# georghess/neurad-studio

Measured on NVIDIA H100. Metric: rays/sec (camera+lidar), higher is better.
Workload: dtype f32

## Files before the change

### neurad-studio_b200/csrc/b200nerf.cu

```cuda
#include <cuda_runtime.h>

#include <cstdio>
#include <cstring>
#include <new>
#include <string>
#include <vector>

#include "../../include/b200nerf.h"
#include "nff_device.h"
#include "nff_lane.h"
#include "rgb_decoder.cuh"
#include "modules.cuh"
#include "lidar_eval.cuh"
#include "lidar_loss.cuh"
#include "image_metrics.cuh"
#include "camera_rays.h"

using namespace nff;

static thread_local std::string g_err;
static int fail(int code, const std::string& msg) {
  g_err = msg;
  return code;
}
// ... 171 lines not shown
  constexpr int kPatchesPerUnit = kLaneThreads / 32;
  return lane_unit_ray(P, patch / kPatchesPerUnit, (int)(patch % kPatchesPerUnit) * 32 + lane_, ray_out);
}

#ifndef NFF_SAMPLE_CTAS
#define NFF_SAMPLE_CTAS 2
#endif
template <int LAYOUT, bool ACTORS, bool TRACED, bool EDIT>
__global__ void __launch_bounds__(kLaneThreads, NFF_SAMPLE_CTAS) nff_sample_lane_kernel(const __grid_constant__ RenderParams P,
                                                                                        float* __restrict__ scratch,
                                                                                        float* __restrict__ handoff) {
  const int tid = threadIdx.x, warp = __shfl_sync(0xffffffffu, (int)(threadIdx.x >> 5), 0), lane_ = tid & 31;
  const LaneScratch sc = lane_scratch_of(scratch, blockIdx.x);
  __shared__ float e0_tab[kS0 + 1];
  const bool shared_edges = !P.rays.nears && !P.rays.fars;
  if (shared_edges) {
    if (tid <= kS0) e0_tab[tid] = lane_round0_edge(P.samp, tid);
    __syncthreads();
  }
  constexpr int kPPU = kLaneThreads / 32;
  const int64_t n_patches = lane_patches(P);
  const int64_t full_rounds = n_patches / kPPU / gridDim.x;
  const int64_t r0 = full_rounds * gridDim.x * kPPU, rest = n_patches - r0;
  const int64_t p0 = r0 + rest * blockIdx.x / gridDim.x, p1 = r0 + rest * (blockIdx.x + 1) / gridDim.x;
  for (int64_t it = 0;; ++it) {
    int64_t patch;
    if (it < full_rounds) {
      patch = (it * gridDim.x + blockIdx.x) * kPPU + warp;
    } else {
      patch = p0 + warp + (it - full_rounds) * kPPU;
      if (patch >= p1) break;
    }
    int64_t ray;
    const bool active = lane_patch_ray(P, patch, lane_, &ray);
    const LaneRay R = lane_ray_setup<ACTORS, EDIT>(P, sc, tid, ray);
    float* col = active ? handoff + ray : sc.bins2 + tid;
    sample_ray_lane<LAYOUT, ACTORS, TRACED>(P, sc, R, tid, ray, active, col, active ? P.n_rays : (int64_t)kLaneThreads,
                                            shared_edges ? e0_tab : nullptr);
  }
}
template <int LAYOUT>
static auto sample_lane_kernel(bool actors, bool traced, bool edit) {
  if (edit) return traced ? nff_sample_lane_kernel<LAYOUT, true, true, true> : nff_sample_lane_kernel<LAYOUT, true, false, true>;
  return traced ? nff_sample_lane_kernel<LAYOUT, true, true, false>
         : actors ? nff_sample_lane_kernel<LAYOUT, true, false, false>
                  : nff_sample_lane_kernel<LAYOUT, false, false, false>;
}

template <int LAYOUT, bool EDIT>
__global__ void __launch_bounds__(kLaneThreads, kLaneCtasPerSm) nff_shade_lane_kernel(const __grid_constant__ RenderParams P,
                                                                                      float* __restrict__ scratch,
                                                                                      const float* __restrict__ handoff) {
  extern __shared__ __align__(128) unsigned char smem_shade[];
  TcShared* tcs = reinterpret_cast<TcShared*>(smem_shade);
  const int tid = threadIdx.x, warp = __shfl_sync(0xffffffffu, (int)(threadIdx.x >> 5), 0), group = warp >> 2;
  tc_stage_weights(*tcs, P.main_mlp_nn, tid, kLaneThreads, true);
  tc::fence_async_smem();
  __syncthreads();
  MlpLaneTc mlp;
  mlp.t = tcs;
  mlp.panel_ = reinterpret_cast<float*>(smem_shade + kTcBytes);
  mlp.bar_id = 1 + group;
  const LaneScratch sc = lane_scratch_of(scratch, blockIdx.x);
  mlp.sh_tcnn = LAYOUT;
  constexpr int kPPU = kLaneThreads / 32;
  const int64_t n_patches = lane_patches(P);
  const int64_t full_rounds = n_patches / kPPU / gridDim.x;
  const int64_t r0 = full_rounds * gridDim.x * kPPU;
  const int64_t rest_groups = (n_patches - r0 + 3) / 4;
  const int64_t g0 = rest_groups * blockIdx.x / gridDim.x, g1 = rest_groups * (blockIdx.x + 1) / gridDim.x;
  for (int64_t it = 0;; ++it) {
    int64_t patch;
    if (it < full_rounds) {
      patch = (it * gridDim.x + blockIdx.x) * kPPU + warp;
    } else {
      const int64_t gu = g0 + group + (it - full_rounds) * (kLaneThreads / 128);
      if (gu >= g1) break;
      patch = r0 + gu * 4 + (warp & 3);
    }
    int64_t ray;
    const bool active = lane_patch_ray(P, patch, tid & 31, &ray);
    const LaneRay R = lane_ray_setup<true, EDIT>(P, sc, tid, ray);
    shade_ray_lane<MlpLaneTc, LAYOUT>(P, sc, R, mlp, tid, ray, active, handoff + ray, P.n_rays);
  }
}

template <bool EDIT>
__global__ void __launch_bounds__(kLaneThreads, kLaneCtasPerSm) nff_render_lane_kernel(const __grid_constant__ RenderParams P,
                                                                          float* __restrict__ scratch) {
  extern __shared__ __align__(128) unsigned char smem_lane[];
  TcShared* tcs = reinterpret_cast<TcShared*>(smem_lane);
  const int tid = threadIdx.x, warp = __shfl_sync(0xffffffffu, (int)(threadIdx.x >> 5), 0), group = warp >> 2;
  tc_stage_weights(*tcs, P.main_mlp_nn, tid, kLaneThreads, true);
  tc::fence_async_smem();
  __syncthreads();
  MlpLaneTc mlp;
  mlp.t = tcs;
  mlp.panel_ = reinterpret_cast<float*>(smem_lane + kTcBytes);
  mlp.bar_id = 1 + group;
  const LaneScratch sc = lane_scratch_of(scratch, blockIdx.x);
  for (int64_t unit = blockIdx.x; unit < lane_units(P); unit += gridDim.x) {
    int64_t ray;
    const bool active = lane_unit_ray(P, unit, tid, &ray);
    render_ray_lane<MlpLaneTc, 0, EDIT>(P, sc, mlp, tid, ray, active);
  }
}

__global__ void lidar_decode_kernel(const float* __restrict__ mlp, const float* __restrict__ feats, int fdim,
                                    int64_t n, float* __restrict__ intensity, float* __restrict__ drop) {
  __shared__ __align__(16) float w[kLidarMlpFloats];
  for (int i = threadIdx.x; i < kLidarMlpFloats; i += blockDim.x) w[i] = mlp[i];
  __syncthreads();
  int64_t r = (int64_t)blockIdx.x * blockDim.x + threadIdx.x;
  if (r >= n) return;
  float x[kNff + kApp];
#pragma unroll
  for (int i = 0; i < kNff + kApp; ++i) x[i] = i < fdim ? feats[r * fdim + i] : 0.f;
  float h[kHidden], h2[kHidden], o[2];
  dense<kNff + kApp, kHidden, kHidden, true>(w + kOffLidW0, w + kOffLidB0, x, h);
  dense<kHidden, kHidden, kHidden, true>(w + kOffLidW1, w + kOffLidB1, h, h2);
  dense<kHidden, 2, kLidOutP, false>(w + kOffLidW2, w + kOffLidB2, h2, o);
  if (intensity) intensity[r] = 1.0f / (1.0f + expf(-o[0]));
  if (drop) drop[r] = o[1];
}

__global__ void hashgrid_fwd_kernel(Grid g, const float* __restrict__ x, float* __restrict__ out,
                                    int32_t* __restrict__ indices, int64_t n_points) {
  int64_t i = (int64_t)blockIdx.x * blockDim.x + threadIdx.x;
  if (i >= n_points * g.L) return;
  int64_t p = i / g.L;
  int l = (int)(i % g.L);
  Cell c = grid_cell(x[3 * p], x[3 * p + 1], x[3 * p + 2], g.res[l]);
  uint32_t r[8];
  cell_rows(c, g.mask, r);
  if (indices) {
#pragma unroll
    for (int k = 0; k < 8; ++k) indices[(p * g.L + l) * 8 + k] = (int32_t)(r[k] + (uint32_t)l * g.T);
  }
  const float* base = g.table + (size_t)l * g.T * g.F;
  for (int f = 0; f < g.F; ++f) {
    float v[8];
#pragma unroll
    for (int k = 0; k < 8; ++k) v[k] = __ldg(base + (size_t)r[k] * g.F + f);
    out[p * g.L * g.F + l * g.F + f] = trilerp(v, c);
  }
}

template <int D>
__global__ void tcnn_hashgrid_fwd_kernel(Grid g, const float* __restrict__ x, float* __restrict__ out, int64_t n) {
  const int64_t i = (int64_t)blockIdx.x * blockDim.x + threadIdx.x;
  if (i >= n) return;
// ... 1750 lines not shown
  const Step steps[10] = {
      {features, nullptr, lo[0], H, W},
      {lo[0], nullptr, lo[1], H, W}, {lo[1], lo[0], lo[2], H, W},
      {lo[2], nullptr, lo[1], H, W}, {lo[1], lo[2], lo[0], H, W},
      {lo[0], nullptr, hi[0], H, W},
      {hi[0], nullptr, hi[1], HO, WO}, {hi[1], hi[0], hi[2], HO, WO},
      {hi[2], nullptr, hi[1], HO, WO}, {hi[1], hi[2], rgb, HO, WO},
  };
  for (int layer = 0; layer < 10; ++layer) {
    const Step& s = steps[layer];
    if (int e = b200nerf_rgb_decode_layer(c, layer, s.in, s.res, s.out, batch, s.h, s.w, impl, stream)) return e;
  }
  return 0;
}

int b200nerf_set_peer_outputs(b200nerf_ctx* c, const b200nerf_peer_outputs* peers) {
  REQUIRE(c, "ctx is NULL");
  if (!peers || peers->n_peers == 0) {
    c->peers = b200nerf_peer_outputs{};
    return 0;
  }
  REQUIRE(peers->n_peers > 0 && peers->n_peers <= B200NERF_MAX_PEERS, "n_peers must be in [1, 16]");
  REQUIRE(peers->self_rank >= -1 && peers->self_rank < peers->n_peers, "self_rank out of range");
  REQUIRE(peers->row_offset >= 0, "negative row_offset");
  for (int p = 0; p < peers->n_peers; ++p) {
    if (p == peers->self_rank) continue;
    REQUIRE(peers->features[p] && peers->depth[p] && peers->accumulation[p], "NULL peer buffer");
  }
  c->peers = *peers;
  return 0;
}

int b200nerf_set_param_stream(b200nerf_ctx* c, void* stream) {
  REQUIRE(c, "ctx is NULL");
  c->param_stream = (cudaStream_t)stream;
  return 0;
}

int b200nerf_set_mlp_mode(b200nerf_ctx* c, int mode) {
  REQUIRE(c, "ctx is NULL");
  REQUIRE(mode >= 0 && mode <= 3, "render mode: 0 = warp-per-ray + CUDA-core fp32, 1 = warp-per-ray + wgmma, 2 = ray-per-lane + wgmma, 3 = ray-per-lane in two kernels (sampling, shading)");
  c->mlp_mode = mode;
  return 0;
}

int b200nerf_check_status(b200nerf_ctx* c) {
  REQUIRE(c, "ctx is NULL");
  if (!c->d_status) return 0;
  DeviceGuard g(c->device);
  int st = 0;
  CUDA_TRY(cudaMemcpy(&st, c->d_status, sizeof(int), cudaMemcpyDeviceToHost));
  if (st != 0) {
    cudaMemset(c->d_status, 0, sizeof(int));
    return fail(B200NERF_ERR_CUDA, "device-side failure flag set (tensor-core pipeline timed out, code " + std::to_string(st) + ")");
  }
  return 0;
}

int b200nerf_hashgrid_fwd(b200nerf_ctx* c, const b200nerf_grid_desc* desc, const float* table, const float* x,
                          float* out, int32_t* indices, int64_t n_points, void* stream) {
  REQUIRE(c && desc, "NULL argument");
  REQUIRE(desc->features_per_level >= 1 && desc->features_per_level <= 8, "features_per_level must be in [1,8]");
  if (n_points == 0) return 0;
  REQUIRE(table && x && out, "NULL argument");
  DeviceGuard g(c->device);
  Grid gr{};
  if (int e = make_grid(desc, table, &gr)) return e;
  if (indices && (uint64_t)gr.L * gr.T > (1ull << 31))
    return fail(B200NERF_ERR_UNSUPPORTED, "row indices of more than 2^31 table rows do not fit int32");
  int64_t n = n_points * gr.L;
  hashgrid_fwd_kernel<<<(unsigned)((n + 255) / 256), 256, 0, (cudaStream_t)stream>>>(gr, x, out, indices, n_points);
  CUDA_TRY(cudaGetLastError());
  return 0;
}

int b200nerf_tcnn_hashgrid_fwd(b200nerf_ctx* c, const b200nerf_tcnn_grid_desc* desc, const float* params, const float* x,
                               float* out, int64_t n_points, void* stream) {
  REQUIRE(c && desc, "NULL argument");
  REQUIRE(desc->features_per_level >= 1 && desc->features_per_level <= 8, "features_per_level must be in [1,8]");
  REQUIRE(desc->n_input_dims == 3 || desc->n_input_dims == 4, "n_input_dims must be 3 or 4");
  if (n_points == 0) return 0;
  REQUIRE(params && x && out, "NULL argument");
  DeviceGuard g(c->device);
  Grid gr{};
  if (int e = make_tcnn_grid(desc, params, desc->n_input_dims, &gr)) return e;
  const unsigned blocks = (unsigned)((n_points + 127) / 128);
  if (desc->n_input_dims == 3)
    tcnn_hashgrid_fwd_kernel<3><<<blocks, 128, 0, (cudaStream_t)stream>>>(gr, x, out, n_points);
  else
    tcnn_hashgrid_fwd_kernel<4><<<blocks, 128, 0, (cudaStream_t)stream>>>(gr, x, out, n_points);
  CUDA_TRY(cudaGetLastError());
  return 0;
}

int b200nerf_sh4_fwd(b200nerf_ctx* c, const float* dirs, float* out, int64_t n, void* stream) {
  REQUIRE(c, "NULL argument");
  if (n == 0) return 0;
  REQUIRE(dirs && out, "NULL argument");
  DeviceGuard g(c->device);
  sh4_fwd_kernel<<<(unsigned)((n + 255) / 256), 256, 0, (cudaStream_t)stream>>>(dirs, out, n);
  CUDA_TRY(cudaGetLastError());
  return 0;
}

int b200nerf_pdf_resample(b200nerf_ctx* c, const float* weights, const float* bins, const float* u, int n_rays,
                          int s_old, int s_new, float hist_pad, float* new_bins, float* cdf, int32_t* inds,
// ... 316 lines not shown
```

### neurad-studio_b200/csrc/nff_device.h

```cpp
#pragma once
#include "nff_params.h"
#include "simt.h"

#ifndef NFF_G_PROP
#define NFF_G_PROP 1
#endif
#ifndef NFF_G_ACT
#define NFF_G_ACT 2
#endif
#ifndef NFF_ILP
#define NFF_ILP 2
#endif
#ifndef NFF_F4_UNROLL
#define NFF_F4_UNROLL 2
#endif
#ifndef NFF_FAST_RCP
#define NFF_FAST_RCP 1
#endif
#ifndef NFF_PARITY_STD
#define NFF_PARITY_STD 0
#endif
#ifndef NFF_PARITY_LERP
#define NFF_PARITY_LERP 0
#endif
// ... 726 lines not shown
struct MlpFfma {
  const float* w;
  template <class WS>
  NFF_D void run(WS& ws, const float dir[3], float& sdf, float* feat) const {
    const int ln = lane();
    const float* mlp = w;
    float mac[kGeoOutP];
    dense_panel<kGeoIn, kHidden, kHidden>(mlp + kOffGeoW0, mlp + kOffGeoB0, ws.act, mac);
#pragma unroll
    for (int i = 0; i < kHidden; ++i) ws.act[i][ln] = fmaxf(mac[i], 0.0f);
    dense_panel<kHidden, kNff + 1, kGeoOutP>(mlp + kOffGeoW1, mlp + kOffGeoB1, ws.act, mac);
    sdf = mac[0];
    float geo[kNff];
#pragma unroll
    for (int i = 0; i < kNff; ++i) {
      geo[i] = mac[i + 1];
      ws.act[i][ln] = geo[i];
    }
    {
      float shv[kSh];
      sh4(dir[0], dir[1], dir[2], shv);
#pragma unroll
      for (int i = 0; i < kSh; ++i) ws.act[kNff + i][ln] = shv[i];
    }
    dense_panel<kNff + kSh, kHidden, kHidden>(mlp + kOffFeatW0, mlp + kOffFeatB0, ws.act, mac);
#pragma unroll
    for (int i = 0; i < kHidden; ++i) ws.act[i][ln] = fmaxf(mac[i], 0.0f);
    dense_panel<kHidden, kHidden, kHidden>(mlp + kOffFeatW1, mlp + kOffFeatB1, ws.act, mac);
#pragma unroll
    for (int i = 0; i < kHidden; ++i) ws.act[i][ln] = fmaxf(mac[i], 0.0f);
    dense_panel<kHidden, kNff, kNff>(mlp + kOffFeatW2, mlp + kOffFeatB2, ws.act, mac);
#pragma unroll
    for (int i = 0; i < kNff; ++i) feat[i] = geo[i] + mac[i];
  }
};

#if defined(__CUDACC__)
}
#include "tc_mlp.cuh"
namespace nff {
constexpr int kTcLayers = 5;
constexpr int kTcPitch = tc::stage_pitch(48);
constexpr int kTcStageFloats = 128 * kTcPitch;
struct TcShared {
  float b[2 * 32 * (32 + 32 + 48 + 32 + 32)];
  float bias[kTcLayers][32];
  float w_sdf[32];
  float b_sdf;
};
constexpr int kTcBytes = (sizeof(TcShared) + 127) / 128 * 128;
constexpr size_t tc_smem_bytes(int threads) { return (size_t)kTcBytes + (size_t)(threads / 128) * kTcStageFloats * sizeof(float); }
NFF_D constexpr int tc_layer_k(int l) { return l == 2 ? 48 : 32; }
NFF_D constexpr int tc_layer_off(int l) { return l == 0 ? 0 : l == 1 ? 2048 : l == 2 ? 4096 : l == 3 ? 7168 : 9216; }

NFF_D void tc_stage_weights(TcShared& t, const float* NFF_RESTRICT nn, int tid, int nthreads, bool chained = false) {
  const int w_off[kTcLayers] = {kNnGeoW0, kNnGeoW1 + kHidden , kNnFeatW0, kNnFeatW1, kNnFeatW2};
  const int b_off[kTcLayers] = {kNnGeoB0, kNnGeoB1 + 1, kNnFeatB0, kNnFeatB1, kNnFeatB2};
#pragma unroll
  for (int l = 0; l < kTcLayers; ++l) {
    const int K = tc_layer_k(l);
    float* hi = t.b + tc_layer_off(l);
    tc::stage_b_tile(hi, hi + 32 * K, nn + w_off[l], 32, K, 32, K, tid, nthreads, chained && l > 0 ? 32 : 0);
    for (int i = tid; i < 32; i += nthreads) t.bias[l][i] = nn[b_off[l] + i];
  }
  for (int i = tid; i < 32; i += nthreads) t.w_sdf[i] = nn[kNnGeoW1 + i];
  if (tid == 0) t.b_sdf = nn[kNnGeoB1];
}

struct MlpTc {
  const TcShared* t;
  float* stage;
  int bar_id;

  template <int K>
  NFF_D void layer(int l, const float* x, float* out) {
    const float* hi = t->b + tc_layer_off(l);
    const int id = bar_id;
    tc::tile_layer<48, 32>(stage, kTcPitch, x, K, hi, hi + 32 * K, out, [id] { asm volatile("bar.sync %0, 128;" ::"r"(id) : "memory"); });
#pragma unroll
    for (int i = 0; i < 32; ++i) out[i] += t->bias[l][i];
  }

  template <class WS>
  NFF_D void run(WS& ws, const float dir[3], float& sdf, float* feat) {
    const int ln = lane();
    float x[kNff + kSh], h[kHidden];
#pragma unroll
    for (int i = 0; i < kGeoIn; ++i) x[i] = ws.act[i][ln];
    layer<32>(0, x, h);
    float s = t->b_sdf;
#pragma unroll
    for (int i = 0; i < kHidden; ++i) {
      h[i] = fmaxf(h[i], 0.0f);
      s = fmaf(h[i], t->w_sdf[i], s);
    }
    sdf = s;
    layer<32>(1, h, x);
    sh4(dir[0], dir[1], dir[2], x + kNff);
    layer<48>(2, x, h);
#pragma unroll
    for (int i = 0; i < kHidden; ++i) h[i] = fmaxf(h[i], 0.0f);
    float h2[kHidden];
    layer<32>(3, h, h2);
#pragma unroll
    for (int i = 0; i < kHidden; ++i) h2[i] = fmaxf(h2[i], 0.0f);
    layer<32>(4, h2, h);
#pragma unroll
    for (int i = 0; i < kNff; ++i) feat[i] = x[i] + h[i];
  }
};
#endif

template <class WS, class Mlp>
NFF_D void render_ray(const RenderParams& P, WS& ws, Mlp& mlp, int64_t ray, bool active) {
  const Sampling& sp = P.samp;
  const int ln = lane();
// ... 127 lines not shown
```

### neurad-studio_b200/csrc/nff_lane.h

```cpp
#pragma once
#include "nff_device.h"

namespace nff {

#ifndef NFF_LANE_THREADS
#define NFF_LANE_THREADS 512
#endif
#ifndef NFF_F4_WEIGHTS
#define NFF_F4_WEIGHTS 0
#endif
constexpr int kLaneThreads = NFF_LANE_THREADS;
constexpr int kLaneCtasPerSm = 512 / kLaneThreads;
constexpr int kCandFloats = 16;
constexpr int kLaneMaxCand = 32;

struct LaneScratch {
  float* w;
  float* bins1;
  float* bins2;
  float* cand;
};
NFF_HD size_t lane_scratch_floats_per_cta() {
  return (size_t)kLaneThreads * (kS0 + (kS1 + 1) + (kS2 + 1) + kLaneMaxCand * kCandFloats);
}
// ... 227 lines not shown
  int k = 1;
  double run = (double)fdiv(fadd(sc.w[tid], pad_each), tot);
  float c_km1 = 0.0f, c_k = fminf(1.0f, (float)run);
  float w_next = sc.w[(size_t)kLaneThreads + tid];
#pragma unroll 1
  for (int i = 0; i <= S_new; ++i) {
    const float u = ldg(io.u_tab + i);
    while (k <= S && c_k <= u) {
      ++k;
      c_km1 = c_k;
      if (k <= S) {
        const float wk = w_next;
        w_next = sc.w[(size_t)(k < S ? k : S - 1) * kLaneThreads + tid];
        run += (double)fdiv(fadd(wk, pad_each), tot);
        c_k = fminf(1.0f, (float)run);
      }
    }
    const int above = k > S ? S : k;
    const float b0 = edge(k - 1), b1 = edge(above);
    float t = nan_to_num(fdiv(fsub(u, c_km1), fsub(k > S ? c_km1 : c_k, c_km1)));
    t = fminf(fmaxf(t, 0.0f), 1.0f);
    const float nb = fadd(b0, fmul(t, fsub(b1, b0)));
    io.bins_out[(size_t)i * io.bins_stride] = nb;
    if (TRACED && io.tr_inds) io.tr_inds[ray * (S_new + 1) + i] = k;
    if (TRACED && io.tr_bins_s) io.tr_bins_s[ray * (S_new + 1) + i] = nb;
    if (TRACED && io.tr_bins_e) io.tr_bins_e[ray * (S_new + 1) + i] = to_euclid(nb, s_near, s_far, sp);
  }
  return depth_acc;
}

struct MlpLaneFfma {
  static constexpr int kPitch = kLaneThreads;
  const float* w;
  float* panel_;
  int sh_tcnn = 0;
  NFF_D float* panel() const { return panel_; }
  NFF_D void run(const float* x, const float dir[3], float& sdf, float* feat, int ) const {
    float h[kHidden], go[kNff + 1], in2[kNff + kSh], h2[kHidden];
    dense<kGeoIn, kHidden, kHidden, true>(w + kOffGeoW0, w + kOffGeoB0, x, h);
    dense<kHidden, kNff + 1, kGeoOutP, false>(w + kOffGeoW1, w + kOffGeoB1, h, go);
    sdf = go[0];
#pragma unroll
    for (int i = 0; i < kNff; ++i) in2[i] = go[i + 1];
    if (sh_tcnn) sh4_tcnn(dir[0], dir[1], dir[2], in2 + kNff); else sh4(dir[0], dir[1], dir[2], in2 + kNff);
    dense<kNff + kSh, kHidden, kHidden, true>(w + kOffFeatW0, w + kOffFeatB0, in2, h);
    dense<kHidden, kHidden, kHidden, true>(w + kOffFeatW1, w + kOffFeatB1, h, h2);
    dense<kHidden, kNff, kNff, false>(w + kOffFeatW2, w + kOffFeatB2, h2, h);
#pragma unroll
    for (int i = 0; i < kNff; ++i) feat[i] = in2[i] + h[i];
  }
};

#if defined(__CUDACC__)
constexpr int kLanePanelPitch = kLaneThreads + 8;
constexpr int kLanePanelRows = kGeoIn + kSh + 1;
constexpr size_t lane_tc_smem_bytes() { return (size_t)kTcBytes + sizeof(float) * kLanePanelRows * kLanePanelPitch; }
struct MlpLaneTc {
  static constexpr int kPitch = kLanePanelPitch;
  const TcShared* t;
  float* panel_;
  int bar_id;
  int sh_tcnn = 0;
  NFF_D float* panel() const { return panel_; }
  NFF_D void group_sync() const { asm volatile("bar.sync %0, 128;" ::"r"(bar_id) : "memory"); }

  NFF_D static uint32_t b_desc_lo() {
    extern __shared__ __align__(128) unsigned char nff_lane_smem[];
    return tc::smem_desc_lo(tc::smem_u32(nff_lane_smem + offsetof(TcShared, b)), 128u);
  }

  template <int KS, int K, int OFF>
  NFF_D static void half_mma(float* acc, const float* a) {
    uint32_t ah[4 * KS], al[4 * KS];
#pragma unroll
    for (int i = 0; i < 4 * KS; ++i) {
      const float h = tc::tf32_hi(a[i]);
      ah[i] = __float_as_uint(h);
      al[i] = __float_as_uint(a[i] - h);
    }
    constexpr uint32_t sbo = (uint32_t)(K / 4) * 128u;
    constexpr uint32_t hi_off = (uint32_t)OFF * 4u / 16u, lo_off = (uint32_t)(OFF + 32 * K) * 4u / 16u;
    const uint32_t b_desc = b_desc_lo();
    tc::wg_fence();
#pragma unroll
    for (int ks = 0; ks < KS; ++ks) {
      const uint32_t adv = (uint32_t)(ks * 2 * 128) / 16u;
      const uint64_t dh = tc::smem_desc_of(b_desc + hi_off + adv, sbo), dl = tc::smem_desc_of(b_desc + lo_off + adv, sbo);
      tc::wgmma_tf32<32>(acc, ah + 4 * ks, dh);
      tc::wgmma_tf32<32>(acc, al + 4 * ks, dh);
      tc::wgmma_tf32<32>(acc, ah + 4 * ks, dl);
    }
    tc::wg_commit();
    tc::wg_wait<0>();
    tc::reg_fence(acc, 16);
#pragma unroll
    for (int i = 0; i < 4 * KS; ++i) asm volatile("" : "+r"(ah[i]), "+r"(al[i])::"memory");
  }
  NFF_D static void chain(float* a, const float* acc) {
#pragma unroll
    for (int j = 0; j < 4; ++j) {
      a[4 * j + 0] = acc[4 * j + 0];
      a[4 * j + 1] = acc[4 * j + 2];
      a[4 * j + 2] = acc[4 * j + 1];
      a[4 * j + 3] = acc[4 * j + 3];
    }
  }
  NFF_D static void load_a(float* a, const float* p, int q, int ks0, int n) {
#pragma unroll
    for (int i = 0; i < n; ++i) {
      const float* r = p + (8 * (ks0 + i) + q) * kPitch;
      a[4 * i + 0] = r[0];
      a[4 * i + 1] = r[8];
      a[4 * i + 2] = r[4 * kPitch];
      a[4 * i + 3] = r[4 * kPitch + 8];
    }
  }
  NFF_D static void bias_init(float* acc, const float* bias, int q) {
#pragma unroll
    for (int j = 0; j < 4; ++j) {
      const float2 b = *reinterpret_cast<const float2*>(bias + 8 * j + 2 * q);
      acc[4 * j + 0] = acc[4 * j + 2] = b.x;
      acc[4 * j + 1] = acc[4 * j + 3] = b.y;
    }
  }
  NFF_D static void relu(float* acc) {
#pragma unroll
    for (int i = 0; i < 16; ++i) acc[i] = fmaxf(acc[i], 0.0f);
  }

  NFF_D void run(const float* , const float dir[3], float& sdf, float* feat, int tid) {
    float* col = panel_ + tid;
    {
      float shv[kSh];
      if (sh_tcnn) sh4_tcnn(dir[0], dir[1], dir[2], shv); else sh4(dir[0], dir[1], dir[2], shv);
#pragma unroll
      for (int i = 0; i < kSh; ++i) col[(kGeoIn + i) * kPitch] = shv[i];
    }
    group_sync();
    const int ln = tid & 31, q = ln & 3;
    float* const fr = panel_ + (tid & ~127) + 16 * ((tid >> 5) & 3) + (ln >> 2);
#pragma unroll 1
    for (int h = 0; h < 2; ++h) {
      float* const p = fr + 64 * h;
      float a[16], acc[16];
      load_a(a, p, q, 0, 4);
      bias_init(acc, t->bias[0], q);
      half_mma<4, 32, tc_layer_off(0)>(acc, a);
      relu(acc);
      float s0 = 0.0f, s1 = 0.0f;
#pragma unroll
      for (int j = 0; j < 4; ++j) {
        const float2 w = *reinterpret_cast<const float2*>(t->w_sdf + 8 * j + 2 * q);
        s0 = fmaf(acc[4 * j + 0], w.x, fmaf(acc[4 * j + 1], w.y, s0));
        s1 = fmaf(acc[4 * j + 2], w.x, fmaf(acc[4 * j + 3], w.y, s1));
      }
      s0 += __shfl_xor_sync(0xffffffffu, s0, 1);
      s1 += __shfl_xor_sync(0xffffffffu, s1, 1);
      s0 += __shfl_xor_sync(0xffffffffu, s0, 2);
      s1 += __shfl_xor_sync(0xffffffffu, s1, 2);
      if (q == 0) {
        p[(kGeoIn + kSh) * kPitch] = s0 + t->b_sdf;
        p[(kGeoIn + kSh) * kPitch + 8] = s1 + t->b_sdf;
      }
      chain(a, acc);
      bias_init(acc, t->bias[1], q);
      half_mma<4, 32, tc_layer_off(1)>(acc, a);
      __syncwarp();
#pragma unroll
      for (int j = 0; j < 4; ++j) {
        float* r = p + (8 * j + 2 * q) * kPitch;
        r[0] = acc[4 * j + 0], r[kPitch] = acc[4 * j + 1], r[8] = acc[4 * j + 2], r[kPitch + 8] = acc[4 * j + 3];
      }
      chain(a, acc);
      bias_init(acc, t->bias[2], q);
      half_mma<4, 48, tc_layer_off(2)>(acc, a);
      load_a(a, p, q, 4, 2);
      half_mma<2, 48, tc_layer_off(2) + 4 * 64>(acc, a);
      relu(acc);
      chain(a, acc);
      bias_init(acc, t->bias[3], q);
      half_mma<4, 32, tc_layer_off(3)>(acc, a);
      relu(acc);
      chain(a, acc);
      bias_init(acc, t->bias[4], q);
#pragma unroll
      for (int j = 0; j < 4; ++j) {
        const float* r = p + (8 * j + 2 * q) * kPitch;
        acc[4 * j + 0] += r[0], acc[4 * j + 1] += r[kPitch], acc[4 * j + 2] += r[8], acc[4 * j + 3] += r[kPitch + 8];
      }
      half_mma<4, 32, tc_layer_off(4)>(acc, a);
#pragma unroll
      for (int j = 0; j < 4; ++j) {
        float* r = p + (8 * j + 2 * q) * kPitch;
        r[0] = acc[4 * j + 0], r[kPitch] = acc[4 * j + 1], r[8] = acc[4 * j + 2], r[kPitch + 8] = acc[4 * j + 3];
      }
    }
    group_sync();
#pragma unroll
    for (int i = 0; i < kNff; ++i) feat[i] = col[i * kPitch];
    sdf = col[(kGeoIn + kSh) * kPitch];
  }
};
#endif

struct LaneRay {
  float o[3], d[3];
  float area, time, s_near, s_far;
  int n_cand;
};
constexpr float kDefaultNear = 0.0f, kDefaultFar = 1.0e6f;
NFF_D void lane_spacing_bounds(const Sampling& sp, float near_, float far_, float* s_near, float* s_far) {
  *s_near = spacing_fn(near_, sp);
  *s_far = spacing_fn(fminf(far_, sp.sky_distance), sp);
}
NFF_D float lane_round0_edge(const Sampling& sp, int i) {
  float s_near, s_far;
  lane_spacing_bounds(sp, kDefaultNear, kDefaultFar, &s_near, &s_far);
  return to_euclid(linspace01(i, kS0), s_near, s_far, sp);
}
template <bool ACTORS = true, bool EDIT = false>
NFF_D LaneRay lane_ray_setup(const RenderParams& P, const LaneScratch& sc, int tid, int64_t ray) {
  const Sampling& sp = P.samp;
  LaneRay R;
#pragma unroll
  for (int i = 0; i < 3; ++i) {
    R.o[i] = ldg(P.rays.origins + 3 * ray + i);
    R.d[i] = ldg(P.rays.directions + 3 * ray + i);
  }
  const bool lidar = P.rays.is_lidar ? P.rays.is_lidar[ray] != 0 : false;
  R.area = fmul(ldg(P.rays.pixel_area + ray), lidar ? 1.0f : sp.cam_area_scale);
  R.time = ldg(P.rays.times + ray);
  const float far_ = P.rays.fars ? ldg(P.rays.fars + ray) : kDefaultFar;
  const float near_ = P.rays.nears ? ldg(P.rays.nears + ray) : kDefaultNear;
  lane_spacing_bounds(sp, near_, far_, &R.s_near, &R.s_far);
  int overflow = 0;
  R.n_cand = ACTORS ? lane_actor_candidates<EDIT>(P.actors, R.time, R.o, R.d, sc, tid, &overflow) : 0;
#if defined(__CUDACC__)
  if (overflow && P.status) atomicExch(P.status, 3);
#endif
  return R;
}

template <int LAYOUT = 0, bool ACTORS = true, bool TRACED = true>
NFF_D void sample_ray_lane(const RenderParams& P, const LaneScratch& sc, const LaneRay& R, int tid, int64_t ray, bool active,
                           float* bins2, int64_t bins2_stride, const float* e0_tab = nullptr) {
  const Sampling& sp = P.samp;
#pragma unroll 1
// ... 190 lines not shown
```

### neurad-studio_b200/csrc/tc_mlp.cuh

```cuda
#pragma once
#include <cuda_runtime.h>
#include <stdint.h>

namespace tc {

__device__ __forceinline__ uint32_t smem_u32(const void* p) { return (uint32_t)__cvta_generic_to_shared(p); }

__device__ __forceinline__ void fence_async_smem() { asm volatile("fence.proxy.async.shared::cta;" ::: "memory"); }
__device__ __forceinline__ void wg_fence() { asm volatile("wgmma.fence.sync.aligned;" ::: "memory"); }
__device__ __forceinline__ void wg_commit() { asm volatile("wgmma.commit_group.sync.aligned;" ::: "memory"); }
template <int N>
__device__ __forceinline__ void wg_wait() { asm volatile("wgmma.wait_group.sync.aligned %0;" ::"n"(N) : "memory"); }
__device__ __forceinline__ void reg_fence(float* d, int n) {
  for (int i = 0; i < n; ++i) asm volatile("" : "+f"(d[i])::"memory");
}

__device__ __forceinline__ void mbar_init(uint64_t* bar, uint32_t count) {
  asm volatile("mbarrier.init.shared::cta.b64 [%0], %1;" ::"r"(smem_u32(bar)), "r"(count) : "memory");
  asm volatile("fence.mbarrier_init.release.cluster;" ::: "memory");
}
__device__ __forceinline__ bool mbar_wait(uint64_t* bar, uint32_t parity) {
  const uint32_t addr = smem_u32(bar);
  for (int it = 0; it < (1 << 20); ++it) {
    uint32_t ok;
    asm volatile(
        "{\n\t.reg .pred p;\n\t"
        "mbarrier.try_wait.parity.shared::cta.b64 p, [%1], %2;\n\t"
        "selp.b32 %0, 1, 0, p;\n\t}"
        : "=r"(ok)
        : "r"(addr), "r"(parity)
        : "memory");
    if (ok) return true;
  }
  return false;
}
__device__ __forceinline__ uint32_t elect_one() {
  uint32_t pred;
  asm volatile(
      "{\n\t.reg .pred P;\n\t"
      "elect.sync _|P, 0xffffffff;\n\t"
      "selp.b32 %0, 1, 0, P;\n\t}"
      : "=r"(pred));
  return pred;
}

#define TC_D8(i) "+f"(d[i]), "+f"(d[i + 1]), "+f"(d[i + 2]), "+f"(d[i + 3]), "+f"(d[i + 4]), "+f"(d[i + 5]), "+f"(d[i + 6]), "+f"(d[i + 7])
#define TC_D16(i) TC_D8(i), TC_D8(i + 8)
#define TC_D32(i) TC_D16(i), TC_D16(i + 16)
__device__ __forceinline__ void wgmma_tf32_m64n16(float* d, const uint32_t* a, uint64_t b_desc) {
  asm volatile("{\n\t.reg .pred p;\n\tsetp.ne.b32 p, %13, 0;\n\twgmma.mma_async.sync.aligned.m64n16k8.f32.tf32.tf32 "
               "{%0, %1, %2, %3, %4, %5, %6, %7}, {%8, %9, %10, %11}, %12, p, 1, 1;\n\t}"
               : TC_D8(0)
               : "r"(a[0]), "r"(a[1]), "r"(a[2]), "r"(a[3]), "l"(b_desc), "r"(1));
}
__device__ __forceinline__ void wgmma_tf32_m64n32(float* d, const uint32_t* a, uint64_t b_desc) {
  asm volatile("{\n\t.reg .pred p;\n\tsetp.ne.b32 p, %21, 0;\n\twgmma.mma_async.sync.aligned.m64n32k8.f32.tf32.tf32 "
               "{%0, %1, %2, %3, %4, %5, %6, %7, %8, %9, %10, %11, %12, %13, %14, %15}, {%16, %17, %18, %19}, %20, p, 1, 1;\n\t}"
               : TC_D16(0)
               : "r"(a[0]), "r"(a[1]), "r"(a[2]), "r"(a[3]), "l"(b_desc), "r"(1));
}
__device__ __forceinline__ void wgmma_tf32_m64n48(float* d, const uint32_t* a, uint64_t b_desc) {
  asm volatile("{\n\t.reg .pred p;\n\tsetp.ne.b32 p, %29, 0;\n\twgmma.mma_async.sync.aligned.m64n48k8.f32.tf32.tf32 "
               "{%0, %1, %2, %3, %4, %5, %6, %7, %8, %9, %10, %11, %12, %13, %14, %15, %16, %17, %18, %19, %20, %21, %22, %23}, {%24, %25, %26, %27}, %28, p, 1, 1;\n\t}"
               : TC_D16(0), TC_D8(16)
               : "r"(a[0]), "r"(a[1]), "r"(a[2]), "r"(a[3]), "l"(b_desc), "r"(1));
}
__device__ __forceinline__ void wgmma_tf32_m64n64(float* d, const uint32_t* a, uint64_t b_desc) {
  asm volatile("{\n\t.reg .pred p;\n\tsetp.ne.b32 p, %37, 0;\n\twgmma.mma_async.sync.aligned.m64n64k8.f32.tf32.tf32 "
               "{%0, %1, %2, %3, %4, %5, %6, %7, %8, %9, %10, %11, %12, %13, %14, %15, %16, %17, %18, %19, %20, %21, %22, %23, %24, %25, %26, %27, %28, %29, %30, %31}, {%32, %33, %34, %35}, %36, p, 1, 1;\n\t}"
               : TC_D32(0)
               : "r"(a[0]), "r"(a[1]), "r"(a[2]), "r"(a[3]), "l"(b_desc), "r"(1));
}
__device__ __forceinline__ void wgmma_bf16_m64n32(float* d, uint64_t a_desc, uint64_t b_desc) {
  asm volatile("{\n\t.reg .pred p;\n\tsetp.ne.b32 p, %18, 0;\n\twgmma.mma_async.sync.aligned.m64n32k16.f32.bf16.bf16 "
               "{%0, %1, %2, %3, %4, %5, %6, %7, %8, %9, %10, %11, %12, %13, %14, %15}, %16, %17, p, 1, 1, 0, 0;\n\t}"
               : TC_D16(0)
               : "l"(a_desc), "l"(b_desc), "r"(1));
}
__device__ __forceinline__ void wgmma_bf16_m64n64(float* d, uint64_t a_desc, uint64_t b_desc) {
  asm volatile("{\n\t.reg .pred p;\n\tsetp.ne.b32 p, %34, 0;\n\twgmma.mma_async.sync.aligned.m64n64k16.f32.bf16.bf16 "
               "{%0, %1, %2, %3, %4, %5, %6, %7, %8, %9, %10, %11, %12, %13, %14, %15, %16, %17, %18, %19, %20, %21, %22, %23, %24, %25, %26, %27, %28, %29, %30, %31}, %32, %33, p, 1, 1, 0, 0;\n\t}"
               : TC_D32(0)
               : "l"(a_desc), "l"(b_desc), "r"(1));
}
__device__ __forceinline__ void wgmma_bf16_m64n96(float* d, uint64_t a_desc, uint64_t b_desc) {
  asm volatile("{\n\t.reg .pred p;\n\tsetp.ne.b32 p, %50, 0;\n\twgmma.mma_async.sync.aligned.m64n96k16.f32.bf16.bf16 "
               "{%0, %1, %2, %3, %4, %5, %6, %7, %8, %9, %10, %11, %12, %13, %14, %15, %16, %17, %18, %19, %20, %21, %22, %23, %24, %25, %26, %27, %28, %29, %30, %31, %32, %33, %34, %35, %36, %37, %38, %39, %40, %41, %42, %43, %44, %45, %46, %47}, %48, %49, p, 1, 1, 0, 0;\n\t}"
               : TC_D32(0), TC_D16(32)
               : "l"(a_desc), "l"(b_desc), "r"(1));
}
__device__ __forceinline__ void wgmma_bf16_m64n128(float* d, uint64_t a_desc, uint64_t b_desc) {
  asm volatile("{\n\t.reg .pred p;\n\tsetp.ne.b32 p, %66, 0;\n\twgmma.mma_async.sync.aligned.m64n128k16.f32.bf16.bf16 "
               "{%0, %1, %2, %3, %4, %5, %6, %7, %8, %9, %10, %11, %12, %13, %14, %15, %16, %17, %18, %19, %20, %21, %22, %23, %24, %25, %26, %27, %28, %29, %30, %31, %32, %33, %34, %35, %36, %37, %38, %39, %40, %41, %42, %43, %44, %45, %46, %47, %48, %49, %50, %51, %52, %53, %54, %55, %56, %57, %58, %59, %60, %61, %62, %63}, %64, %65, p, 1, 1, 0, 0;\n\t}"
               : TC_D32(0), TC_D32(32)
               : "l"(a_desc), "l"(b_desc), "r"(1));
}
template <int N>
__device__ __forceinline__ void wgmma_tf32(float* d, const uint32_t* a, uint64_t b_desc) {
  static_assert(N == 16 || N == 32 || N == 48 || N == 64, "tf32 tile widths");
  if constexpr (N == 16) wgmma_tf32_m64n16(d, a, b_desc);
  else if constexpr (N == 32) wgmma_tf32_m64n32(d, a, b_desc);
  else if constexpr (N == 48) wgmma_tf32_m64n48(d, a, b_desc);
  else wgmma_tf32_m64n64(d, a, b_desc);
}

__host__ __device__ constexpr uint32_t b_tile_floats(int n_pad, int k_pad) { return (uint32_t)(n_pad * k_pad); }
__device__ __forceinline__ uint32_t b_elem_offset(int n, int k, int k_pad) {
  return (uint32_t)((n >> 3) * (k_pad >> 2) * 32 + (k >> 2) * 32 + (n & 7) * 4 + (k & 3));
}
__device__ __forceinline__ float tf32_hi(float x) { return __uint_as_float(__float_as_uint(x) & 0xffffe000u); }

__host__ __device__ constexpr int chained_k(int k) { return (k & ~7) | ((k & 7) < 4 ? 2 * (k & 7) : 2 * (k & 7) - 7); }

__device__ __forceinline__ void stage_b_tile(float* hi, float* lo, const float* __restrict__ w, int n_real, int k_real, int n_pad,
                                             int k_pad, int tid, int nthreads, int k_chained = 0) {
  for (int i = tid; i < n_pad * k_pad; i += nthreads) {
    int n = i / k_pad, k = i % k_pad;
    const int kw = k < k_chained ? chained_k(k) : k;
    float v = (n < n_real && kw < k_real) ? w[n * k_real + kw] : 0.0f;
    float h = tf32_hi(v);
    uint32_t off = b_elem_offset(n, k, k_pad);
    hi[off] = h;
    lo[off] = v - h;
  }
}
__device__ __forceinline__ uint64_t smem_desc(uint32_t saddr, uint32_t lbo_bytes, uint32_t sbo_bytes) {
  return (uint64_t)((saddr & 0x3ffffu) >> 4) | ((uint64_t)(lbo_bytes >> 4) << 16) | ((uint64_t)(sbo_bytes >> 4) << 32);
}
__device__ __forceinline__ uint32_t smem_desc_lo(uint32_t saddr, uint32_t lbo_bytes) {
  return ((saddr & 0x3ffffu) >> 4) | ((lbo_bytes >> 4) << 16);
}
__device__ __forceinline__ uint64_t smem_desc_of(uint32_t lo, uint32_t sbo_bytes) {
  return (uint64_t)lo | ((uint64_t)(sbo_bytes >> 4) << 32);
}

__host__ __device__ constexpr int stage_pitch(int w) { return (w + 7) / 8 * 8 + 4; }

template <int K_MAX>
__device__ __forceinline__ void store_row(float* stage, int pitch, const float* x, int n) {
  float4* dst = reinterpret_cast<float4*>(stage + (threadIdx.x & 127) * pitch);
#pragma unroll
  for (int c = 0; c < K_MAX; c += 4)
    if (c < n) dst[c / 4] = make_float4(x[c], x[c + 1], x[c + 2], x[c + 3]);
}
template <int N_MAX>
__device__ __forceinline__ void load_row(const float* stage, int pitch, float* y, int n) {
  const float4* src = reinterpret_cast<const float4*>(stage + (threadIdx.x & 127) * pitch);
#pragma unroll
  for (int c = 0; c < N_MAX; c += 4)
    if (c < n) {
      const float4 v = src[c / 4];
      y[c] = v.x, y[c + 1] = v.y, y[c + 2] = v.z, y[c + 3] = v.w;
    }
}

template <int N>
__device__ __forceinline__ void tile_mma(const float* stage, int pitch, int k_pad, const float* b_hi, const float* b_lo, float* acc) {
  const int wq = (threadIdx.x >> 5) & 3, ln = threadIdx.x & 31, g = ln >> 2, t = ln & 3;
  const uint32_t sbo = (uint32_t)(k_pad >> 2) * 128u;
  const uint64_t dh0 = smem_desc(smem_u32(b_hi), 128u, sbo), dl0 = smem_desc(smem_u32(b_lo), 128u, sbo);
  for (int ks = 0; ks < k_pad / 8; ++ks) {
    uint32_t ah[2][4], al[2][4];
#pragma unroll
    for (int h = 0; h < 2; ++h) {
      const float* r0 = stage + (64 * h + 16 * wq + g) * pitch + 8 * ks + t;
      const float* r1 = r0 + 8 * pitch;
      const float v[4] = {r0[0], r1[0], r0[4], r1[4]};
#pragma unroll
      for (int i = 0; i < 4; ++i) {
        const float vh = tf32_hi(v[i]);
        ah[h][i] = __float_as_uint(vh);
        al[h][i] = __float_as_uint(v[i] - vh);
      }
    }
    const uint64_t adv = (uint64_t)((ks * 2 * 128) >> 4);
    wg_fence();
// ... 44 lines not shown
```

Before: 87.62 million.

## Switch lane-mode shading MLP from split-tf32 to scaled split-fp16 wgmma

The ray-per-lane MLP used three tf32 wgmma (k8) per k-step with hi/lo operand splits. It now uses fp16 hi/lo splits with k16 wgmma, which halves the number of k-steps. Weights are rescaled per layer by a power of two derived from the layer's max absolute weight, and activations by a fixed factor of 64, to keep values inside fp16 range. An overflow check writes a device status code when an activation gets too large. This adds scaling multiplies, a per-layer max reduction at weight staging, and a risk of range errors or accuracy loss.

```diff
diff --git a/neurad-studio_b200/csrc/b200nerf.cu b/neurad-studio_b200/csrc/b200nerf.cu
--- a/neurad-studio_b200/csrc/b200nerf.cu
+++ b/neurad-studio_b200/csrc/b200nerf.cu
@@ -247,14 +247,15 @@
                                                                                       float* __restrict__ scratch,
                                                                                       const float* __restrict__ handoff) {
   extern __shared__ __align__(128) unsigned char smem_shade[];
-  TcShared* tcs = reinterpret_cast<TcShared*>(smem_shade);
+  LaneTcShared* tcs = reinterpret_cast<LaneTcShared*>(smem_shade);
   const int tid = threadIdx.x, warp = __shfl_sync(0xffffffffu, (int)(threadIdx.x >> 5), 0), group = warp >> 2;
-  tc_stage_weights(*tcs, P.main_mlp_nn, tid, kLaneThreads, true);
+  lane_tc_stage_weights(*tcs, P.main_mlp_nn, tid, kLaneThreads);
   tc::fence_async_smem();
   __syncthreads();
   MlpLaneTc mlp;
   mlp.t = tcs;
-  mlp.panel_ = reinterpret_cast<float*>(smem_shade + kTcBytes);
+  mlp.panel_ = reinterpret_cast<float*>(smem_shade + kLaneTcBytes);
+  mlp.status = P.status;
   mlp.bar_id = 1 + group;
   const LaneScratch sc = lane_scratch_of(scratch, blockIdx.x);
   mlp.sh_tcnn = LAYOUT;
@@ -284,14 +285,15 @@
 __global__ void __launch_bounds__(kLaneThreads, kLaneCtasPerSm) nff_render_lane_kernel(const __grid_constant__ RenderParams P,
                                                                           float* __restrict__ scratch) {
   extern __shared__ __align__(128) unsigned char smem_lane[];
-  TcShared* tcs = reinterpret_cast<TcShared*>(smem_lane);
+  LaneTcShared* tcs = reinterpret_cast<LaneTcShared*>(smem_lane);
   const int tid = threadIdx.x, warp = __shfl_sync(0xffffffffu, (int)(threadIdx.x >> 5), 0), group = warp >> 2;
-  tc_stage_weights(*tcs, P.main_mlp_nn, tid, kLaneThreads, true);
+  lane_tc_stage_weights(*tcs, P.main_mlp_nn, tid, kLaneThreads);
   tc::fence_async_smem();
   __syncthreads();
   MlpLaneTc mlp;
   mlp.t = tcs;
-  mlp.panel_ = reinterpret_cast<float*>(smem_lane + kTcBytes);
+  mlp.panel_ = reinterpret_cast<float*>(smem_lane + kLaneTcBytes);
+  mlp.status = P.status;
   mlp.bar_id = 1 + group;
   const LaneScratch sc = lane_scratch_of(scratch, blockIdx.x);
   for (int64_t unit = blockIdx.x; unit < lane_units(P); unit += gridDim.x) {
@@ -2148,6 +2150,10 @@
   CUDA_TRY(cudaMemcpy(&st, c->d_status, sizeof(int), cudaMemcpyDeviceToHost));
   if (st != 0) {
     cudaMemset(c->d_status, 0, sizeof(int));
+    if (st == kLaneTcRangeStatus)
+      return fail(B200NERF_ERR_CUDA, "device-side failure flag set (code " + std::to_string(st) +
+                                         "): a main-field MLP activation reached the fp16 operand range of the shading "
+                                         "tensor cores (|x| >= 1023.75)");
     return fail(B200NERF_ERR_CUDA, "device-side failure flag set (tensor-core pipeline timed out, code " + std::to_string(st) + ")");
   }
   return 0;
diff --git a/neurad-studio_b200/csrc/nff_device.h b/neurad-studio_b200/csrc/nff_device.h
--- a/neurad-studio_b200/csrc/nff_device.h
+++ b/neurad-studio_b200/csrc/nff_device.h
@@ -802,16 +802,16 @@
 constexpr size_t tc_smem_bytes(int threads) { return (size_t)kTcBytes + (size_t)(threads / 128) * kTcStageFloats * sizeof(float); }
 NFF_D constexpr int tc_layer_k(int l) { return l == 2 ? 48 : 32; }
 NFF_D constexpr int tc_layer_off(int l) { return l == 0 ? 0 : l == 1 ? 2048 : l == 2 ? 4096 : l == 3 ? 7168 : 9216; }
-
-NFF_D void tc_stage_weights(TcShared& t, const float* NFF_RESTRICT nn, int tid, int nthreads, bool chained = false) {
-  const int w_off[kTcLayers] = {kNnGeoW0, kNnGeoW1 + kHidden , kNnFeatW0, kNnFeatW1, kNnFeatW2};
-  const int b_off[kTcLayers] = {kNnGeoB0, kNnGeoB1 + 1, kNnFeatB0, kNnFeatB1, kNnFeatB2};
+NFF_D constexpr int tc_layer_w(int l) { return l == 0 ? kNnGeoW0 : l == 1 ? kNnGeoW1 + kHidden : l == 2 ? kNnFeatW0 : l == 3 ? kNnFeatW1 : kNnFeatW2; }
+NFF_D constexpr int tc_layer_b(int l) { return l == 0 ? kNnGeoB0 : l == 1 ? kNnGeoB1 + 1 : l == 2 ? kNnFeatB0 : l == 3 ? kNnFeatB1 : kNnFeatB2; }
+
+NFF_D void tc_stage_weights(TcShared& t, const float* NFF_RESTRICT nn, int tid, int nthreads) {
 #pragma unroll
   for (int l = 0; l < kTcLayers; ++l) {
     const int K = tc_layer_k(l);
     float* hi = t.b + tc_layer_off(l);
-    tc::stage_b_tile(hi, hi + 32 * K, nn + w_off[l], 32, K, 32, K, tid, nthreads, chained && l > 0 ? 32 : 0);
-    for (int i = tid; i < 32; i += nthreads) t.bias[l][i] = nn[b_off[l] + i];
+    tc::stage_b_tile(hi, hi + 32 * K, nn + tc_layer_w(l), 32, K, 32, K, tid, nthreads);
+    for (int i = tid; i < 32; i += nthreads) t.bias[l][i] = nn[tc_layer_b(l) + i];
   }
   for (int i = tid; i < 32; i += nthreads) t.w_sdf[i] = nn[kNnGeoW1 + i];
   if (tid == 0) t.b_sdf = nn[kNnGeoB1];
diff --git a/neurad-studio_b200/csrc/nff_lane.h b/neurad-studio_b200/csrc/nff_lane.h
--- a/neurad-studio_b200/csrc/nff_lane.h
+++ b/neurad-studio_b200/csrc/nff_lane.h
@@ -303,13 +303,55 @@
 };
 
 #if defined(__CUDACC__)
-constexpr int kLanePanelPitch = kLaneThreads + 8;
+constexpr int kLanePanelPitch = kLaneThreads + 4;
 constexpr int kLanePanelRows = kGeoIn + kSh + 1;
-constexpr size_t lane_tc_smem_bytes() { return (size_t)kTcBytes + sizeof(float) * kLanePanelRows * kLanePanelPitch; }
+constexpr int kLaneTcA = 6;
+constexpr float kLaneTcAScale = 64.0f, kLaneTcAUnscale = 1.0f / 64.0f;
+constexpr float kLaneTcOverflow = 65520.0f;
+constexpr int kLaneTcRangeStatus = 4;
+struct LaneTcShared {
+  __half b[2 * 32 * (32 + 32 + 48 + 32 + 32)];
+  float bias[kTcLayers][32];
+  float up[kTcLayers], down[kTcLayers];
+  float w_sdf[32];
+  float b_sdf;
+  unsigned wmax[kTcLayers];
+};
+constexpr int kLaneTcBytes = (sizeof(LaneTcShared) + 127) / 128 * 128;
+constexpr size_t lane_tc_smem_bytes() { return (size_t)kLaneTcBytes + sizeof(float) * kLanePanelRows * kLanePanelPitch; }
+
+NFF_D void lane_tc_stage_weights(LaneTcShared& t, const float* NFF_RESTRICT nn, int tid, int nthreads) {
+  if (tid < kTcLayers) t.wmax[tid] = 0u;
+  __syncthreads();
+#pragma unroll
+  for (int l = 0; l < kTcLayers; ++l) {
+    unsigned m = 0u;
+    for (int i = tid; i < 32 * tc_layer_k(l); i += nthreads) m = max(m, __float_as_uint(fabsf(nn[tc_layer_w(l) + i])));
+    m = __reduce_max_sync(0xffffffffu, m);
+    if ((tid & 31) == 0 && m) atomicMax(&t.wmax[l], m);
+  }
+  __syncthreads();
+#pragma unroll
+  for (int l = 0; l < kTcLayers; ++l) {
+    int E;
+    frexpf(__uint_as_float(t.wmax[l]), &E);
+    const int e = min(max(15 - E, -60), 60);
+    const float up = __int_as_float((127 + e) << 23), down = __int_as_float((127 - e) << 23);
+    const int K = tc_layer_k(l);
+    __half* hi = t.b + tc_layer_off(l);
+    tc::stage_b_tile_f16(hi, hi + 32 * K, nn + tc_layer_w(l), K, up, tid, nthreads);
+    for (int i = tid; i < 32; i += nthreads) t.bias[l][i] = nn[tc_layer_b(l) + i] * up * kLaneTcAScale;
+    if (tid == 0) t.up[l] = up, t.down[l] = down;
+  }
+  for (int i = tid; i < 32; i += nthreads) t.w_sdf[i] = nn[kNnGeoW1 + i];
+  if (tid == 0) t.b_sdf = nn[kNnGeoB1];
+}
+
 struct MlpLaneTc {
   static constexpr int kPitch = kLanePanelPitch;
-  const TcShared* t;
+  const LaneTcShared* t;
   float* panel_;
+  int* status;
   int bar_id;
   int sh_tcnn = 0;
   NFF_D float* panel() const { return panel_; }
@@ -317,29 +359,30 @@
 
   NFF_D static uint32_t b_desc_lo() {
     extern __shared__ __align__(128) unsigned char nff_lane_smem[];
-    return tc::smem_desc_lo(tc::smem_u32(nff_lane_smem + offsetof(TcShared, b)), 128u);
+    return tc::smem_desc_lo(tc::smem_u32(nff_lane_smem + offsetof(LaneTcShared, b)), 128u);
   }
 
   template <int KS, int K, int OFF>
-  NFF_D static void half_mma(float* acc, const float* a) {
+  NFF_D void half_mma(float* acc, const float* a) const {
     uint32_t ah[4 * KS], al[4 * KS];
+    float amax = 0.0f;
 #pragma unroll
     for (int i = 0; i < 4 * KS; ++i) {
-      const float h = tc::tf32_hi(a[i]);
-      ah[i] = __float_as_uint(h);
-      al[i] = __float_as_uint(a[i] - h);
-    }
-    constexpr uint32_t sbo = (uint32_t)(K / 4) * 128u;
-    constexpr uint32_t hi_off = (uint32_t)OFF * 4u / 16u, lo_off = (uint32_t)(OFF + 32 * K) * 4u / 16u;
+      amax = fmaxf(amax, fmaxf(fabsf(a[2 * i]), fabsf(a[2 * i + 1])));
+      tc::f16x2_split(a[2 * i], a[2 * i + 1], ah[i], al[i]);
+    }
+    if (amax >= kLaneTcOverflow && status) atomicExch(status, kLaneTcRangeStatus);
+    constexpr uint32_t sbo = (uint32_t)(K / 8) * 128u;
+    constexpr uint32_t hi_off = (uint32_t)OFF * 2u / 16u, lo_off = (uint32_t)(OFF + 32 * K) * 2u / 16u;
     const uint32_t b_desc = b_desc_lo();
     tc::wg_fence();
 #pragma unroll
     for (int ks = 0; ks < KS; ++ks) {
       const uint32_t adv = (uint32_t)(ks * 2 * 128) / 16u;
       const uint64_t dh = tc::smem_desc_of(b_desc + hi_off + adv, sbo), dl = tc::smem_desc_of(b_desc + lo_off + adv, sbo);
-      tc::wgmma_tf32<32>(acc, ah + 4 * ks, dh);
-      tc::wgmma_tf32<32>(acc, al + 4 * ks, dh);
-      tc::wgmma_tf32<32>(acc, ah + 4 * ks, dl);
+      tc::wgmma_f16_m64n32(acc, ah + 4 * ks, dh);
+      tc::wgmma_f16_m64n32(acc, al + 4 * ks, dh);
+      tc::wgmma_f16_m64n32(acc, ah + 4 * ks, dl);
     }
     tc::wg_commit();
     tc::wg_wait<0>();
@@ -347,23 +390,18 @@
 #pragma unroll
     for (int i = 0; i < 4 * KS; ++i) asm volatile("" : "+r"(ah[i]), "+r"(al[i])::"memory");
   }
-  NFF_D static void chain(float* a, const float* acc) {
-#pragma unroll
-    for (int j = 0; j < 4; ++j) {
-      a[4 * j + 0] = acc[4 * j + 0];
-      a[4 * j + 1] = acc[4 * j + 2];
-      a[4 * j + 2] = acc[4 * j + 1];
-      a[4 * j + 3] = acc[4 * j + 3];
-    }
-  }
   NFF_D static void load_a(float* a, const float* p, int q, int ks0, int n) {
 #pragma unroll
     for (int i = 0; i < n; ++i) {
-      const float* r = p + (8 * (ks0 + i) + q) * kPitch;
-      a[4 * i + 0] = r[0];
-      a[4 * i + 1] = r[8];
-      a[4 * i + 2] = r[4 * kPitch];
-      a[4 * i + 3] = r[4 * kPitch + 8];
+      const float* r = p + (16 * (ks0 + i) + 2 * q) * kPitch;
+      a[8 * i + 0] = r[0] * kLaneTcAScale;
+      a[8 * i + 1] = r[kPitch] * kLaneTcAScale;
+      a[8 * i + 2] = r[8] * kLaneTcAScale;
+      a[8 * i + 3] = r[kPitch + 8] * kLaneTcAScale;
+      a[8 * i + 4] = r[8 * kPitch] * kLaneTcAScale;
+      a[8 * i + 5] = r[9 * kPitch] * kLaneTcAScale;
+      a[8 * i + 6] = r[8 * kPitch + 8] * kLaneTcAScale;
+      a[8 * i + 7] = r[9 * kPitch + 8] * kLaneTcAScale;
     }
   }
   NFF_D static void bias_init(float* acc, const float* bias, int q) {
@@ -373,6 +411,10 @@
       acc[4 * j + 0] = acc[4 * j + 2] = b.x;
       acc[4 * j + 1] = acc[4 * j + 3] = b.y;
     }
+  }
+  NFF_D static void unscale(float* acc, float down) {
+#pragma unroll
+    for (int i = 0; i < 16; ++i) acc[i] *= down;
   }
   NFF_D static void relu(float* acc) {
 #pragma unroll
@@ -393,10 +435,11 @@
 #pragma unroll 1
     for (int h = 0; h < 2; ++h) {
       float* const p = fr + 64 * h;
-      float a[16], acc[16];
-      load_a(a, p, q, 0, 4);
+      float a[24], acc[16];
+      load_a(a, p, q, 0, 2);
       bias_init(acc, t->bias[0], q);
-      half_mma<4, 32, tc_layer_off(0)>(acc, a);
+      half_mma<2, 32, tc_layer_off(0)>(acc, a);
+      unscale(acc, t->down[0]);
       relu(acc);
       float s0 = 0.0f, s1 = 0.0f;
 #pragma unroll
@@ -410,40 +453,49 @@
       s0 += __shfl_xor_sync(0xffffffffu, s0, 2);
       s1 += __shfl_xor_sync(0xffffffffu, s1, 2);
       if (q == 0) {
-        p[(kGeoIn + kSh) * kPitch] = s0 + t->b_sdf;
-        p[(kGeoIn + kSh) * kPitch + 8] = s1 + t->b_sdf;
-      }
-      chain(a, acc);
+        p[(kGeoIn + kSh) * kPitch] = s0 * kLaneTcAUnscale + t->b_sdf;
+        p[(kGeoIn + kSh) * kPitch + 8] = s1 * kLaneTcAUnscale + t->b_sdf;
+      }
+#pragma unroll
+      for (int i = 0; i < 16; ++i) a[i] = acc[i];
       bias_init(acc, t->bias[1], q);
-      half_mma<4, 32, tc_layer_off(1)>(acc, a);
+      half_mma<2, 32, tc_layer_off(1)>(acc, a);
+      unscale(acc, t->down[1]);
       __syncwarp();
 #pragma unroll
       for (int j = 0; j < 4; ++j) {
         float* r = p + (8 * j + 2 * q) * kPitch;
         r[0] = acc[4 * j + 0], r[kPitch] = acc[4 * j + 1], r[8] = acc[4 * j + 2], r[kPitch + 8] = acc[4 * j + 3];
       }
-      chain(a, acc);
+#pragma unroll
+      for (int i = 0; i < 16; ++i) a[i] = acc[i];
+      load_a(a + 16, p, q, 2, 1);
       bias_init(acc, t->bias[2], q);
-      half_mma<4, 48, tc_layer_off(2)>(acc, a);
-      load_a(a, p, q, 4, 2);
-      half_mma<2, 48, tc_layer_off(2) + 4 * 64>(acc, a);
+      half_mma<3, 48, tc_layer_off(2)>(acc, a);
+      unscale(acc, t->down[2]);
       relu(acc);
-      chain(a, acc);
+#pragma unroll
+      for (int i = 0; i < 16; ++i) a[i] = acc[i];
       bias_init(acc, t->bias[3], q);
-      half_mma<4, 32, tc_layer_off(3)>(acc, a);
+      half_mma<2, 32, tc_layer_off(3)>(acc, a);
+      unscale(acc, t->down[3]);
       relu(acc);
-      chain(a, acc);
+#pragma unroll
+      for (int i = 0; i < 16; ++i) a[i] = acc[i];
       bias_init(acc, t->bias[4], q);
+      const float up4 = t->up[4], out4 = t->down[4] * kLaneTcAUnscale;
 #pragma unroll
       for (int j = 0; j < 4; ++j) {
         const float* r = p + (8 * j + 2 * q) * kPitch;
-        acc[4 * j + 0] += r[0], acc[4 * j + 1] += r[kPitch], acc[4 * j + 2] += r[8], acc[4 * j + 3] += r[kPitch + 8];
-      }
-      half_mma<4, 32, tc_layer_off(4)>(acc, a);
+        acc[4 * j + 0] += r[0] * up4, acc[4 * j + 1] += r[kPitch] * up4;
+        acc[4 * j + 2] += r[8] * up4, acc[4 * j + 3] += r[kPitch + 8] * up4;
+      }
+      half_mma<2, 32, tc_layer_off(4)>(acc, a);
 #pragma unroll
       for (int j = 0; j < 4; ++j) {
         float* r = p + (8 * j + 2 * q) * kPitch;
-        r[0] = acc[4 * j + 0], r[kPitch] = acc[4 * j + 1], r[8] = acc[4 * j + 2], r[kPitch + 8] = acc[4 * j + 3];
+        r[0] = acc[4 * j + 0] * out4, r[kPitch] = acc[4 * j + 1] * out4;
+        r[8] = acc[4 * j + 2] * out4, r[kPitch + 8] = acc[4 * j + 3] * out4;
       }
     }
     group_sync();
diff --git a/neurad-studio_b200/csrc/tc_mlp.cuh b/neurad-studio_b200/csrc/tc_mlp.cuh
--- a/neurad-studio_b200/csrc/tc_mlp.cuh
+++ b/neurad-studio_b200/csrc/tc_mlp.cuh
@@ -1,4 +1,5 @@
 #pragma once
+#include <cuda_fp16.h>
 #include <cuda_runtime.h>
 #include <stdint.h>
 
@@ -95,6 +96,12 @@
                : TC_D32(0), TC_D32(32)
                : "l"(a_desc), "l"(b_desc), "r"(1));
 }
+__device__ __forceinline__ void wgmma_f16_m64n32(float* d, const uint32_t* a, uint64_t b_desc) {
+  asm volatile("{\n\t.reg .pred p;\n\tsetp.ne.b32 p, %21, 0;\n\twgmma.mma_async.sync.aligned.m64n32k16.f32.f16.f16 "
+               "{%0, %1, %2, %3, %4, %5, %6, %7, %8, %9, %10, %11, %12, %13, %14, %15}, {%16, %17, %18, %19}, %20, p, 1, 1, 0;\n\t}"
+               : TC_D16(0)
+               : "r"(a[0]), "r"(a[1]), "r"(a[2]), "r"(a[3]), "l"(b_desc), "r"(1));
+}
 template <int N>
 __device__ __forceinline__ void wgmma_tf32(float* d, const uint32_t* a, uint64_t b_desc) {
   static_assert(N == 16 || N == 32 || N == 48 || N == 64, "tf32 tile widths");
@@ -110,18 +117,37 @@
 }
 __device__ __forceinline__ float tf32_hi(float x) { return __uint_as_float(__float_as_uint(x) & 0xffffe000u); }
 
-__host__ __device__ constexpr int chained_k(int k) { return (k & ~7) | ((k & 7) < 4 ? 2 * (k & 7) : 2 * (k & 7) - 7); }
-
 __device__ __forceinline__ void stage_b_tile(float* hi, float* lo, const float* __restrict__ w, int n_real, int k_real, int n_pad,
-                                             int k_pad, int tid, int nthreads, int k_chained = 0) {
+                                             int k_pad, int tid, int nthreads) {
   for (int i = tid; i < n_pad * k_pad; i += nthreads) {
     int n = i / k_pad, k = i % k_pad;
-    const int kw = k < k_chained ? chained_k(k) : k;
-    float v = (n < n_real && kw < k_real) ? w[n * k_real + kw] : 0.0f;
+    float v = (n < n_real && k < k_real) ? w[n * k_real + k] : 0.0f;
     float h = tf32_hi(v);
     uint32_t off = b_elem_offset(n, k, k_pad);
     hi[off] = h;
     lo[off] = v - h;
+  }
+}
+
+__device__ __forceinline__ void f16x2_split(float x0, float x1, uint32_t& hi, uint32_t& lo) {
+  const __half2 h = __floats2half2_rn(x0, x1);
+  const float2 hf = __half22float2(h);
+  const __half2 l = __floats2half2_rn(x0 - hf.x, x1 - hf.y);
+  hi = *reinterpret_cast<const uint32_t*>(&h);
+  lo = *reinterpret_cast<const uint32_t*>(&l);
+}
+__device__ __forceinline__ uint32_t b_elem_offset_f16(int n, int k, int k_pad) {
+  return (uint32_t)((n >> 3) * (k_pad >> 3) * 64 + (k >> 3) * 64 + (n & 7) * 8 + (k & 7));
+}
+__device__ __forceinline__ void stage_b_tile_f16(__half* hi, __half* lo, const float* __restrict__ w, int k_real, float scale,
+                                                 int tid, int nthreads) {
+  for (int i = tid; i < 32 * k_real; i += nthreads) {
+    const int n = i / k_real, k = i % k_real;
+    const float v = w[i] * scale;
+    const __half h = __float2half_rn(v);
+    const uint32_t off = b_elem_offset_f16(n, k, k_real);
+    hi[off] = h;
+    lo[off] = __float2half_rn(v - __half2float(h));
   }
 }
 __device__ __forceinline__ uint64_t smem_desc(uint32_t saddr, uint32_t lbo_bytes, uint32_t sbo_bytes) {
```

New measurement: 90.54 million, median of 6. 3.3% higher.
